# NVIDIA/spark-rapids-ml

Measured on NVIDIA H100. Metric: kmeans_fit_samples_per_sec, higher is better.
Workload: dtype f32

## Files before the change

### profile_fused.py

```python
from __future__ import annotations

import argparse
import json
import os
import sys

ROOT = os.path.dirname(os.path.abspath(__file__))
if ROOT not in sys.path:
    sys.path.insert(0, ROOT)

from bench_pca import _card

CONSUMER = ["X wait", "centre wait", "hand-off wait", "A load + split", "MMA issue + drain", "epilogue", "sort",
            "column sums"]
PRODUCER = ["X slot wait", "centre stage wait", "issue"]
TILE_ROWS = 128


def main() -> None:
    ap = argparse.ArgumentParser()
    ap.add_argument("--rows", type=int, default=10_000_000)
    ap.add_argument("--d", type=int, default=128)
    ap.add_argument("--k", type=int, default=64)
    ap.add_argument("--warmup", type=int, default=3)
    a = ap.parse_args()

    import numpy as np
    import torch

    from bench import make_blobs_device
    from spark_rapids_ml_b200 import _native

    dev = torch.device("cuda", 0)
    X, _ = make_blobs_device(torch, dev, a.rows, a.d, a.k, 0)
    C0 = X[: a.k].clone()
    with _native.Context(0) as ctx:
        ctx.set_option("kernel_path", 2)
        ctx.kmeans_lloyd(X, C0.clone(), a.warmup, -1.0)
        ctx.set_option("profile_fused", 1)
        ctx.kmeans_lloyd(X, C0.clone(), 1, -1.0)
        ctx.set_option("profile_fused", 0)
        prof = ctx.fused_profile().astype(np.float64)
    grid = prof.shape[0]
    ntiles = -(-a.rows // TILE_ROWS)
    tiles = np.array([len(range(b, ntiles, grid)) for b in range(grid)], dtype=np.float64)
    per_tile = prof / tiles[:, None, None]
    cons = per_tile[:, :8, :].mean(axis=(0, 1))
    prod = per_tile[:, 8, :3].mean(axis=0)
    rec = {"shape": {"n": a.rows, "d": a.d, "k": a.k}, "grid": grid, "tiles_per_cta": float(tiles.mean()),
           "consumer_cycles_per_tile": {nm: round(float(v)) for nm, v in zip(CONSUMER, cons)},
           "consumer_total": round(float(cons.sum())),
           "producer_cycles_per_tile": {nm: round(float(v)) for nm, v in zip(PRODUCER, prod)},
           "producer_total": round(float(prod.sum())), **_card()}
    print(f"{rec['gpu']}, power limit {rec['power_limit']}; grid {grid}, {rec['tiles_per_cta']:.1f} tiles per CTA")
    print("consumer warps (mean), cycles per tile:")
    for nm, v in rec["consumer_cycles_per_tile"].items():
        print(f"  {nm:20s} {v:8d}")
    print(f"  {'total':20s} {rec['consumer_total']:8d}")
    print("producer warp, cycles per tile:")
    for nm, v in rec["producer_cycles_per_tile"].items():
        print(f"  {nm:20s} {v:8d}")
    print(f"  {'total':20s} {rec['producer_total']:8d}")
    print(json.dumps(rec))


if __name__ == "__main__":
    main()
```

### spark_rapids_ml_b200/_native.py

```python
from __future__ import annotations

import ctypes
import os
import subprocess
from typing import Any, Dict, List, Optional, Sequence, Tuple

import numpy as np

_PKG_DIR = os.path.dirname(os.path.abspath(__file__))
LIB_PATH = os.environ.get("B2K_LIB") or os.path.join(_PKG_DIR, "libb2kmeans.so")
CSRC_DIR = os.path.join(_PKG_DIR, "csrc")

B2K_OK = 0
INIT_ARRAY, INIT_RANDOM, INIT_KMEANS_PARALLEL = 0, 1, 2
PATH_AUTO, PATH_GENERIC, PATH_FUSED = 0, 1, 2
LAYOUT_ROWS, LAYOUT_COLUMNS = 0, 1
UNIQUE_ID_BYTES = 128

_DTYPE_CODES = {
    np.dtype("float32"): 0,
    np.dtype("float64"): 1,
    np.dtype("int8"): 2,
    np.dtype("int16"): 3,
    np.dtype("int32"): 4,
# ... 203 lines not shown
    L.b2k_dbscan_fit.argtypes = [vp, vp, i64, i32, f64, i32, i32, vp, vp, ctypes.POINTER(i64), ctypes.c_size_t]
    L.b2k_rf_fit.argtypes = [vp, vp, vp, i64, i32, ctypes.POINTER(RfParams), ctypes.POINTER(i32), ctypes.POINTER(i64),
                             vp, vp, ctypes.c_size_t]
    L.b2k_rf_forest.argtypes = [vp, vp, vp, vp, vp, vp, vp, vp]
    L.b2k_rf_predict.argtypes = [vp, vp, i64, i32, i32, vp, vp, vp, vp, vp, i32, i32, vp, vp, vp, ctypes.c_size_t]
    L.b2k_eval_linear.argtypes = [vp, vp, vp, i64, i32, i32, vp, vp, vp, vp, vp, i32, f64, vp, vp, vp, vp, vp,
                                  ctypes.c_size_t]
    L.b2k_eval_forest.argtypes = [vp, vp, vp, i64, i32, i32, i32, vp, vp, vp, vp, vp, vp, vp, i32, f64, vp, vp, vp, vp,
                                  vp, ctypes.c_size_t]
    L.b2k_eval_linear_scores.argtypes = [vp, vp, vp, i64, i32, i32, vp, vp, vp, vp, vp, i64, vp, ctypes.c_size_t]
    L.b2k_eval_forest_scores.argtypes = [vp, vp, vp, i64, i32, i32, vp, vp, vp, vp, vp, vp, vp, vp, i64, vp,
                                         ctypes.c_size_t]
    L.b2k_eval_binary.argtypes = [vp, vp, vp, i64, i32, i32, i32, vp, ctypes.c_size_t]
    L.b2k_umap_fit.argtypes = [vp, vp, i64, i32, vp, ctypes.POINTER(UmapParams), vp, vp, ctypes.c_size_t]
    L.b2k_umap_graph.argtypes = [vp] + [vp] * 11
    L.b2k_umap_transform.argtypes = [vp, vp, vp, i64, i32, vp, i64, ctypes.POINTER(UmapParams), vp, ctypes.c_size_t]
    for name in EXPORTED_SYMBOLS:
        if name not in ("b2k_last_error",):
            getattr(L, name).restype = i32
    _lib = L
    return L


def comm_unique_id() -> bytes:
    L = load_library()
    buf = ctypes.create_string_buffer(UNIQUE_ID_BYTES)
    rc = L.b2k_comm_unique_id(buf)
    if rc != B2K_OK:
        raise B2KError(rc, (L.b2k_last_error(None) or b"").decode())
    return buf.raw


def pca_finalize(cov: np.ndarray, n_total: int, k: int) -> Dict[str, np.ndarray]:
    L = load_library()
    cov = np.ascontiguousarray(cov, dtype=np.float64)
    if cov.ndim != 2 or cov.shape[0] != cov.shape[1]:
        raise ValueError("cov must be a square matrix")
    d = int(cov.shape[0])
    kk = max(int(k), 0)
    comp = np.zeros((kk, d), dtype=np.float64)
    evr = np.zeros(kk, dtype=np.float64)
    sv = np.zeros(kk, dtype=np.float64)
    rc = L.b2k_pca_finalize(cov.ctypes.data, d, int(n_total), int(k), comp.ctypes.data, evr.ctypes.data, sv.ctypes.data)
    if rc != B2K_OK:
        raise B2KError(rc, (L.b2k_last_error(None) or b"").decode())
    return {"components_": comp, "explained_variance_ratio_": evr, "singular_values_": sv}


def linreg_solve(mean: np.ndarray, moments: np.ndarray, n_total: int, reg: float = 0.0, l1_ratio: float = 0.0,
                 fit_intercept: bool = True, standardization: bool = True, max_iter: int = 100,
                 tol: float = 1e-6) -> Tuple[np.ndarray, float, int]:
    L = load_library()
    mean = np.ascontiguousarray(mean, dtype=np.float64)
    moments = np.ascontiguousarray(moments, dtype=np.float64)
    d = int(mean.shape[0]) - 1
    if mean.ndim != 1 or moments.shape != (d + 1, d + 1):
        raise ValueError("mean must be [d + 1] and moments [d + 1, d + 1]")
    coef = np.zeros(max(d, 0), dtype=np.float64)
    b = ctypes.c_double(0.0)
    it = ctypes.c_int(0)
    rc = L.b2k_linreg_solve(mean.ctypes.data, moments.ctypes.data, d, int(n_total), float(reg), float(l1_ratio),
                            int(bool(fit_intercept)), int(bool(standardization)), int(max_iter), float(tol),
                            coef.ctypes.data, ctypes.byref(b), ctypes.byref(it))
    if rc != B2K_OK:
        raise B2KError(rc, (L.b2k_last_error(None) or b"").decode())
    return coef, float(b.value), int(it.value)


def logreg_minimize(fun: Any, x0: np.ndarray, l1: Optional[np.ndarray] = None, max_iter: int = 100,
                    tol: float = 1e-6) -> Tuple[np.ndarray, int, int, float]:
    L = load_library()
    x = np.array(x0, dtype=np.float64, copy=True)
    n = int(x.shape[0])
    l1a = None if l1 is None else np.ascontiguousarray(l1, dtype=np.float64)
    if l1a is not None and l1a.shape != (n,):
        raise ValueError(f"l1 must be [{n}]")
    err: list = []

    def _cb(_user: Any, m: int, xp: Any, fp: Any, gp: Any) -> int:
        try:
            f, g = fun(np.ctypeslib.as_array(xp, shape=(m,)).copy())
            fp[0] = float(f)
            np.ctypeslib.as_array(gp, shape=(m,))[:] = np.asarray(g, dtype=np.float64)
            return 0
        except Exception as e:
            err.append(e)
            return 1

    cb = LOGREG_OBJECTIVE(_cb)
    it, ev, fv = ctypes.c_int(0), ctypes.c_int(0), ctypes.c_double(0.0)
    rc = L.b2k_logreg_minimize(cb, None, n, x.ctypes.data, l1a.ctypes.data if l1a is not None else None,
                               int(max_iter), float(tol), ctypes.byref(it), ctypes.byref(ev), ctypes.byref(fv))
    if err:
        raise err[0]
    if rc != B2K_OK:
        raise B2KError(rc, (L.b2k_last_error(None) or b"").decode())
    return x, int(it.value), int(ev.value), float(fv.value)


def _stream_handle(torch_mod: Any, device: Any) -> int:
    return int(torch_mod.cuda.current_stream(device).cuda_stream)


class Context:

    def __init__(self, device: int = 0):
        import torch

        self._torch = torch
        self._L = load_library()
        self.device_index = int(device)
        self.device = torch.device("cuda", self.device_index)
        h = ctypes.c_void_p()
        rc = self._L.b2k_ctx_create(self.device_index, ctypes.byref(h))
        if rc != B2K_OK:
            raise B2KError(rc, (self._L.b2k_last_error(None) or b"").decode())
        self._h = h
        self.nranks = 1
        self.rank = 0

    def _check(self, rc: int) -> None:
        if rc != B2K_OK:
            raise B2KError(rc, (self._L.b2k_last_error(self._h) or b"").decode())

    def _stream(self) -> int:
        return _stream_handle(self._torch, self.device)

    def close(self) -> None:
        if getattr(self, "_h", None) is not None and self._h:
            self._L.b2k_ctx_destroy(self._h)
            self._h = None

    def __enter__(self) -> "Context":
        return self

    def __exit__(self, *exc: Any) -> None:
        self.close()

    def __del__(self) -> None:
        try:
            self.close()
        except Exception:
            pass

    def set_option(self, key: str, value: int) -> None:
        self._check(self._L.b2k_ctx_set_option(self._h, key.encode(), int(value)))

    def stats(self) -> Dict[str, Any]:
        st = Stats()
        self._check(self._L.b2k_get_stats(self._h, ctypes.byref(st)))
        return {f: getattr(st, f) for f, _ in Stats._fields_}

    def fused_profile(self) -> "np.ndarray":
        buf = np.zeros(1024 * 32 * 8, dtype=np.int64)
        g, w = ctypes.c_int(0), ctypes.c_int(0)
        self._check(self._L.b2k_get_fused_profile(self._h, buf.ctypes.data, buf.size, ctypes.byref(g), ctypes.byref(w)))
        return buf[: g.value * w.value * 8].reshape(g.value, w.value, 8)

    def reset_stats(self) -> None:
        self._check(self._L.b2k_reset_stats(self._h))

    def comm_init(self, nranks: int, rank: int, uid: bytes) -> None:
        assert len(uid) == UNIQUE_ID_BYTES
        self._check(self._L.b2k_comm_init(self._h, int(nranks), int(rank), uid))
        self.nranks, self.rank = int(nranks), int(rank)

    def comm_destroy(self) -> None:
        self._check(self._L.b2k_comm_destroy(self._h))
        self.nranks, self.rank = 1, 0

    def comm_abort(self) -> None:
        self._check(self._L.b2k_comm_abort(self._h))
        self.nranks, self.rank = 1, 0

    def ingest_rows(self, dst: Any, row0: int, values: np.ndarray, d: int,
                    offsets: Optional[np.ndarray] = None, n_rows: Optional[int] = None) -> int:
        code = _DTYPE_CODES.get(values.dtype)
        if code is None:
            raise TypeError(f"unsupported source dtype {values.dtype}")
        assert values.flags.c_contiguous
        if offsets is not None:
            offsets = np.ascontiguousarray(offsets, dtype=np.int32)
            n_b = offsets.shape[0] - 1
        else:
            n_b = int(n_rows) if n_rows is not None else values.size // d
            if values.size != n_b * d:
                raise ValueError(f"feature batch holds {values.size} values for {n_b} rows of width {d}: "
                                 "row width differs from the expected dimension")
        wrote = ctypes.c_int64(0)
        self._check(self._L.b2k_ingest_append(
            self._h, dst.data_ptr(), int(dst.shape[0]), int(d), int(row0), values.ctypes.data,
            offsets.ctypes.data if offsets is not None else None, int(n_b), code, LAYOUT_ROWS,
            self._stream(), ctypes.byref(wrote)))
        return int(wrote.value)

    def ingest_pinned_tensor(self, dst: Any, row0: int, src: Any) -> int:
        assert src.dtype == self._torch.float32 and src.is_contiguous()
        n_b, d = int(src.shape[0]), int(src.shape[1])
        wrote = ctypes.c_int64(0)
        self._check(self._L.b2k_ingest_append(
            self._h, dst.data_ptr(), int(dst.shape[0]), d, int(row0), src.data_ptr(), None, n_b, 0,
            LAYOUT_ROWS, self._stream(), ctypes.byref(wrote)))
        return int(wrote.value)

    def ingest_columns(self, dst: Any, row0: int, columns: Sequence[np.ndarray]) -> int:
        d = len(columns)
        dt = columns[0].dtype
        code = _DTYPE_CODES.get(dt)
        if code is None:
            raise TypeError(f"unsupported source dtype {dt}")
        n_b = int(columns[0].shape[0])
        cols = [np.ascontiguousarray(c) for c in columns]
        for c in cols:
            if c.dtype != dt or c.shape[0] != n_b:
                raise ValueError("columns must share dtype and length")
        ptrs = (ctypes.c_void_p * d)(*[c.ctypes.data for c in cols])
        wrote = ctypes.c_int64(0)
        self._check(self._L.b2k_ingest_append(
            self._h, dst.data_ptr(), int(dst.shape[0]), d, int(row0), ctypes.addressof(ptrs), None, n_b,
            code, LAYOUT_COLUMNS, self._stream(), ctypes.byref(wrote)))
        self._torch.cuda.current_stream(self.device).synchronize()
        return int(wrote.value)

    def _check_X(self, X: Any) -> Tuple[int, int]:
        t = self._torch
        if not (X.is_cuda and X.dtype == t.float32 and X.dim() == 2 and X.is_contiguous()):
            raise ValueError("X must be a contiguous float32 CUDA tensor [n, d]")
        if X.device.index != self.device_index:
            raise ValueError("X lives on a different device than this context")
        return int(X.shape[0]), int(X.shape[1])

    def kmeans_fit(self, X: Any, k: int, *, init: Any = "scalable-k-means++", max_iter: int = 300,
                   tol: float = 1e-4, seed: int = 0, oversampling_factor: float = 2.0, n_init: int = 1,
                   compute_inertia: bool = True) -> Dict[str, Any]:
        t = self._torch
        n, d = self._check_X(X)
        init_ptr = None
        if isinstance(init, str):
            mode = {"scalable-k-means++": INIT_KMEANS_PARALLEL, "k-means||": INIT_KMEANS_PARALLEL,
                    "random": INIT_RANDOM}.get(init)
            if mode is None:
                raise ValueError(f"unknown init {init!r}")
            keep = None
        else:
            keep = t.as_tensor(init, dtype=t.float32, device=self.device).contiguous()
            if tuple(keep.shape) != (k, d):
                raise ValueError(f"init array must have shape ({k}, {d})")
            mode = INIT_ARRAY
            init_ptr = keep.data_ptr()
        centers = t.empty((k, d), dtype=t.float32, device=self.device)
        n_iter = ctypes.c_int(0)
        inertia = ctypes.c_double(0.0)
        with t.cuda.device(self.device):
            self._check(self._L.b2k_kmeans_fit(
                self._h, X.data_ptr(), n, d, int(k), mode, init_ptr, int(max_iter), float(tol),
                int(seed) & 0xFFFFFFFFFFFFFFFF, float(oversampling_factor), int(n_init), centers.data_ptr(),
                ctypes.byref(n_iter), ctypes.byref(inertia) if compute_inertia else None, self._stream()))
        del keep
        return {"cluster_centers_": centers, "n_iter_": int(n_iter.value),
                "inertia_": float(inertia.value) if compute_inertia else None}

    def kmeans_lloyd(self, X: Any, centers: Any, max_iter: int, tol: float) -> Tuple[int, float]:
        t = self._torch
        n, d = self._check_X(X)
        if not (centers.is_cuda and centers.dtype == t.float32 and centers.is_contiguous()
                and centers.shape[1] == d):
            raise ValueError("centers must be a contiguous float32 CUDA tensor [k, d]")
        n_iter = ctypes.c_int(0)
        shift = ctypes.c_double(0.0)
        with t.cuda.device(self.device):
            self._check(self._L.b2k_kmeans_lloyd(
                self._h, X.data_ptr(), n, d, int(centers.shape[0]), centers.data_ptr(), int(max_iter),
                float(tol), ctypes.byref(n_iter), ctypes.byref(shift), self._stream()))
        return int(n_iter.value), float(shift.value)

    def kmeans_assign(self, X: Any, centers: Any, want_mindist: bool = False) -> Tuple[Any, Any]:
        t = self._torch
        n, d = self._check_X(X)
        C = t.as_tensor(centers, dtype=t.float32, device=self.device).contiguous()
        if C.dim() != 2 or C.shape[1] != d:
            raise ValueError("centers must be [k, d]")
        labels = t.empty((n,), dtype=t.int32, device=self.device)
        md = t.empty((n,), dtype=t.float32, device=self.device) if want_mindist else None
        with t.cuda.device(self.device):
            self._check(self._L.b2k_kmeans_assign(
                self._h, X.data_ptr(), n, d, C.data_ptr(), int(C.shape[0]), labels.data_ptr(),
                md.data_ptr() if md is not None else None, self._stream()))
        t.cuda.current_stream(self.device).synchronize()
        return labels, md

    def pca_fit(self, X: Any, k: int) -> Dict[str, np.ndarray]:
        n, d = self._check_X(X)
        kk = max(int(k), 0)
        mean = np.zeros(d, dtype=np.float64)
        comp = np.zeros((kk, d), dtype=np.float64)
        evr = np.zeros(kk, dtype=np.float64)
        sv = np.zeros(kk, dtype=np.float64)
        with self._torch.cuda.device(self.device):
            self._check(self._L.b2k_pca_fit(self._h, X.data_ptr(), n, d, int(k), mean.ctypes.data, comp.ctypes.data,
                                            evr.ctypes.data, sv.ctypes.data, self._stream()))
        return {"mean_": mean, "components_": comp, "explained_variance_ratio_": evr, "singular_values_": sv}

    def pca_transform(self, X: Any, components: Any) -> Any:
        t = self._torch
        n, d = self._check_X(X)
        C = t.as_tensor(components, dtype=t.float32, device=self.device).contiguous()
        if C.dim() != 2 or C.shape[1] != d:
            raise ValueError(f"components must be [k, {d}]")
        k = int(C.shape[0])
        out = t.empty((n, k), dtype=t.float32, device=self.device)
# ... 416 lines not shown
```

### spark_rapids_ml_b200/csrc/b2k_wg.cuh

```cuda
constexpr int WG_TM = B2K_FUSED_TILE_ROWS;
constexpr int WG_CHUNK = 32;
constexpr int WG_XBYTES = WG_TM * WG_CHUNK * 4;
constexpr int WG_NTHREADS = 384;
constexpr int WG_SMEM_LIMIT = 227 * 1024;
constexpr int WG_MISC = 7680;
constexpr int WG_M_CNORM = 256, WG_M_XN = 1280, WG_M_LAB = 1792, WG_M_FLAG = 2816, WG_M_COST = 2880, WG_M_SRT = 2944,
              WG_M_LIST = 3584;
constexpr int WG_MISC3 = 2368;
constexpr int WG_M3_XN = 768, WG_M3_SRT = 768, WG_M3_HIST = 1280, WG_M3_COST = 2304;
constexpr int WG_CL = 8;
constexpr int WG_NPROF = 8;
enum { WG_P_WX, WG_P_WC, WG_P_HAND, WG_P_SPLIT, WG_P_MMA, WG_P_EPI, WG_P_SORT, WG_P_SUMS };

template <int KP, int NCH, bool THREE, bool UPD>
struct WgCfg {
  static_assert(KP % 16 == 0 && KP >= 16 && KP <= 256, "KP");
  static_assert(!UPD || !THREE || (KP <= 128 && NCH <= 4), "3xTF32 covers k, d <= 128");
  static constexpr int SROWS = THREE ? KP : KP / WG_CL;
  static constexpr int DP = NCH * WG_CHUNK;
  static constexpr int NB = THREE ? 2 : 1;
  static constexpr int CBYTES = KP * WG_CHUNK * 4;
  static constexpr int CSTAGE = NB * CBYTES;
  static constexpr int MISC = THREE ? WG_MISC3 : WG_MISC;
  static constexpr int SUM_BYTES = UPD ? SROWS * DP * 4 + SROWS * 4 : 0;
  static constexpr int FIXED = SUM_BYTES + MISC;
  static constexpr int XMIN = UPD ? NCH : 2;
  static constexpr int XRES = UPD ? 2 * NCH : 2;
  static constexpr bool CRES = THREE && (WG_SMEM_LIMIT - FIXED - NCH * CSTAGE) / WG_XBYTES >= XRES;
  static constexpr int SC = CRES ? 1 : (WG_SMEM_LIMIT - FIXED - 2 * CSTAGE) / WG_XBYTES >= XMIN ? 2 : 1;
  static constexpr int C_BYTES = CRES ? NCH * CSTAGE : SC * CSTAGE;
  static constexpr int SX_RAW = (WG_SMEM_LIMIT - FIXED - C_BYTES) / WG_XBYTES;
  static constexpr int SX = SX_RAW > 12 ? 12 : SX_RAW;
  static_assert(SX >= XMIN && 2 * (SX + SC) * 8 + 16 <= WG_M_CNORM, "ring");
  static constexpr int OFF_X = 0;
  static constexpr int OFF_C = SX * WG_XBYTES;
  static constexpr int OFF_SUM = OFF_C + C_BYTES;
  static constexpr int OFF_MISC = OFF_SUM + (THREE ? (SUM_BYTES + 7) & ~7 : (SUM_BYTES + 1023) & ~1023);
  static constexpr int SMEM_BYTES = OFF_MISC + MISC;
  static_assert(SMEM_BYTES <= WG_SMEM_LIMIT, "smem");
  static_assert(!THREE || WG_M_CNORM + KP * 4 <= WG_M3_XN, "misc");
  static_assert(!THREE || WG_M3_HIST + 8 * KP <= WG_M3_COST, "misc");
};
static_assert(WgCfg<64, 4, true, true>::CRES, "cfg2 centres no longer resident");

struct WgArgs {
  int64_t n;
  int ntiles;
  int k;
  int d;
  const float* cnorm;
  int32_t* labels_out;
  float* mind_out;
  double* cost_partials;
  float* partials;
  int32_t* counts;
  const B2kLoopState* st;
  const float* X;
  const float* C32;
  const float* thr;
  const float2* xnorm;
  int2* fix_list;
  uint32_t* fix_masks;
  int32_t* fix_count;
  int seg_cap;
  int mask_cap;
  unsigned long long* rstat;
  long long* prof;
};

__device__ __forceinline__ void wg_merge2(uint32_t& a1, uint32_t& a2, uint32_t b1, uint32_t b2) {
  const uint32_t lo = min(a1, b1), hi = max(a1, b1);
  a2 = min(hi, min(a2, b2));
  a1 = lo;
}

template <int KP, int NCH, bool THREE, bool NC, bool UPD, bool PROF = false>
__global__ void __launch_bounds__(WG_NTHREADS, 1)
k_wg_assign(const __grid_constant__ CUtensorMap mapX, const __grid_constant__ CUtensorMap mapC0,
            const __grid_constant__ CUtensorMap mapC1, const WgArgs args) {
  using G = WgCfg<KP, NCH, THREE, UPD>;
  constexpr int R = KP / 2;
  constexpr int DP = G::DP;
  if (args.st != nullptr && args.st->done) return;

  extern __shared__ __align__(1024) uint8_t smem_raw[];
  const uint32_t base = smem_u32(smem_raw);
  if ((base & 1023u) != 0u) {
    if (threadIdx.x == 0) printf("b2k wgmma: dynamic shared memory base %u is not 1 KB aligned\n", base);
    __trap();
  }
  uint8_t* misc = smem_raw + G::OFF_MISC;
  const uint32_t bars = base + G::OFF_MISC;
  float* cnorm_s = reinterpret_cast<float*>(misc + WG_M_CNORM);
  float* xn_s = reinterpret_cast<float*>(misc + WG_M3_XN);
  int32_t* lab_s = reinterpret_cast<int32_t*>(misc + WG_M_LAB);
  uint8_t* hist_s = misc + WG_M3_HIST;
  int32_t* flag_s = reinterpret_cast<int32_t*>(misc + WG_M_FLAG);
  double* cost_s = reinterpret_cast<double*>(misc + (THREE ? WG_M3_COST : WG_M_COST));
  uint32_t* srt_s = reinterpret_cast<uint32_t*>(misc + (THREE ? WG_M3_SRT : WG_M_SRT));
  float* sum_s = reinterpret_cast<float*>(smem_raw + G::OFF_SUM);
  int32_t* cnt_s = reinterpret_cast<int32_t*>(sum_s + G::SROWS * DP);
  uint32_t* list_s = reinterpret_cast<uint32_t*>(misc + WG_M_LIST);
  auto xfull = [&](int s) -> uint32_t { return bars + 8u * (uint32_t)s; };
  auto xempty = [&](int s) -> uint32_t { return bars + 8u * (uint32_t)(G::SX + s); };
  auto cfull = [&](int s) -> uint32_t { return bars + 8u * (uint32_t)(2 * G::SX + s); };
  auto cempty = [&](int s) -> uint32_t { return bars + 8u * (uint32_t)(2 * G::SX + G::SC + s); };
  constexpr bool CLU = UPD && !THREE;
  const uint32_t ready_bar = bars + 8u * (uint32_t)(2 * G::SX + 2 * G::SC);
  const uint32_t done_bar = ready_bar + 8u;

  const int warp = threadIdx.x >> 5;
  const int lane = threadIdx.x & 31;
  long long pc[WG_NPROF] = {};
  long long tp = PROF ? clock64() : 0;
  auto mark = [&](int ph) {
    if constexpr (PROF) {
      const long long t = clock64();
      pc[ph] += t - tp;
      tp = t;
    }
  };
  auto prof_store = [&]() {
    if constexpr (PROF) {
      long long* o = args.prof + ((size_t)blockIdx.x * (WG_NTHREADS / 32) + warp) * WG_NPROF;
      for (int i = 0; i < WG_NPROF; ++i) o[i] = pc[i];
    }
  };
  if (threadIdx.x == 0) {
    for (int s = 0; s < G::SX; ++s) {
      mbar_init(xfull(s), 1);
      mbar_init(xempty(s), 8);
    }
    for (int s = 0; s < G::SC; ++s) {
      mbar_init(cfull(s), 1);
      mbar_init(cempty(s), 8);
    }
    if constexpr (CLU) {
      mbar_init(ready_bar, WG_CL);
      mbar_init(done_bar, WG_CL);
    }
    asm volatile("fence.mbarrier_init.release.cluster;" ::: "memory");
  }
  for (int j = threadIdx.x; j < KP; j += WG_NTHREADS) cnorm_s[j] = args.cnorm[j];
  if constexpr (UPD) {
    for (int i = threadIdx.x; i < G::SROWS * DP + G::SROWS; i += WG_NTHREADS) sum_s[i] = 0.f;
  }
  __syncthreads();
  uint32_t crank = 0;
  if constexpr (CLU) {
    crank = cluster_ctarank();
    cluster_sync_all();
  }

  const int b0 = (int)blockIdx.x - (int)crank;
  const int nit = b0 < args.ntiles ? (args.ntiles - 1 - b0) / (int)gridDim.x + 1 : 0;

  if (warp >= 8) {
    if constexpr (!THREE) asm volatile("setmaxnreg.dec.sync.aligned.u32 40;" ::: "memory");
    if (warp == 8 && elect_one()) {
      tma_prefetch_desc(&mapX);
      tma_prefetch_desc(&mapC0);
      if constexpr (THREE) tma_prefetch_desc(&mapC1);
      if constexpr (G::CRES) {
        mbar_expect_tx(cfull(0), (uint32_t)(NCH * G::CSTAGE));
        for (int c = 0; c < NCH; ++c) {
          const uint32_t cst = base + (uint32_t)(G::OFF_C + c * G::CSTAGE);
          tma_load_2d(cst, &mapC0, cfull(0), c * WG_CHUNK, 0);
          tma_load_2d(cst + G::CBYTES, &mapC1, cfull(0), c * WG_CHUNK, 0);
        }
      }
      for (int it = 0; it < nit; ++it) {
        const int tile = (int)blockIdx.x + it * (int)gridDim.x;
#pragma unroll 1
        for (int c = 0; c < NCH; ++c) {
          const int q = it * NCH + c;
          const int xs = q % G::SX, cs = q % G::SC;
          mark(WG_P_HAND);
          mbar_wait_nocall(xempty(xs), (uint32_t)((q / G::SX) & 1) ^ 1u);
          mark(WG_P_WX);
          mbar_expect_tx(xfull(xs), (uint32_t)WG_XBYTES);
          tma_load_2d(base + (uint32_t)(G::OFF_X + xs * WG_XBYTES), &mapX, xfull(xs), c * WG_CHUNK, tile * WG_TM);
          if constexpr (!G::CRES) {
            mark(WG_P_HAND);
            mbar_wait_nocall(cempty(cs), (uint32_t)((q / G::SC) & 1) ^ 1u);
            mark(WG_P_WC);
            const uint32_t cst = base + (uint32_t)(G::OFF_C + cs * G::CSTAGE);
            mbar_expect_tx(cfull(cs), (uint32_t)G::CSTAGE);
            tma_load_2d(cst, &mapC0, cfull(cs), c * WG_CHUNK, 0);
            if constexpr (THREE) tma_load_2d(cst + G::CBYTES, &mapC1, cfull(cs), c * WG_CHUNK, 0);
          }
        }
      }
      mark(WG_P_HAND);
      prof_store();
    }
    __syncwarp();
  } else {
    if constexpr (!THREE) asm volatile("setmaxnreg.inc.sync.aligned.u32 232;" ::: "memory");
    const int g = warp >> 2, wi = warp & 3, tw = threadIdx.x & 127;
    float acc[R];
#pragma unroll
    for (int i = 0; i < R; ++i) acc[i] = 0.f;
    double cost = 0.0;
    int seg_cnt = 0;
    unsigned long long n_flag = 0;
    float thr0 = 0.f, thr1 = 0.f, thr2 = 0.f, thr3 = 0.f;
    if constexpr (!THREE) {
      thr0 = args.thr[0];
      thr1 = args.thr[1];
      thr2 = args.thr[2];
      thr3 = args.thr[3];
    }
    if constexpr (THREE) {
      const uint32_t arow = (uint32_t)(g * 64 + wi * 16 + (lane >> 2)) * 128u + (uint32_t)(lane & 3) * 4u;
      const uint32_t asw = (uint32_t)(lane >> 2);
      constexpr bool PIPE = (G::CRES || G::SC > 1) && KP < 128;
      if constexpr (G::CRES) {
        mark(WG_P_EPI);
        if (nit > 0) mbar_wait_nocall(cfull(0), 0u);
        mark(WG_P_WC);
      }
      for (int it = 0; it < nit; ++it) {
        const int tile = (int)blockIdx.x + it * (int)gridDim.x;
        float xnp[4] = {0.f, 0.f, 0.f, 0.f};
#pragma unroll
        for (int c = 0; c < NCH; ++c) {
          const int q = it * NCH + c;
          const int xsl = q % G::SX, csl = q % G::SC;
          const uint32_t xs = base + (uint32_t)(G::OFF_X + xsl * WG_XBYTES);
          const uint32_t cs = base + (uint32_t)(G::OFF_C + (G::CRES ? c : csl) * G::CSTAGE);
          const uint8_t* xp = smem_raw + G::OFF_X + xsl * WG_XBYTES;
          mark(WG_P_EPI);
          mbar_wait_nocall(xfull(xsl), (uint32_t)((q / G::SX) & 1));
          mark(WG_P_WX);
          if constexpr (NC) {
#pragma unroll
            for (int i = 0; i < 4; ++i) {
              const float4 v = lds128(xs + (uint32_t)(g * (WG_XBYTES / 2) + (tw + 128 * i) * 16));
              xnp[i] = fmaf(v.w, v.w, fmaf(v.z, v.z, fmaf(v.y, v.y, fmaf(v.x, v.x, xnp[i]))));
            }
          }
          uint32_t ah[WG_CHUNK / 8][4], al[WG_CHUNK / 8][4];
#pragma unroll
          for (int ks = 0; ks < WG_CHUNK / 8; ++ks) {
#pragma unroll
            for (int e = 0; e < 4; ++e) {
              const uint32_t unit = (uint32_t)(2 * ks + (e >> 1));
              const float v = *reinterpret_cast<const float*>(xp + arow + (uint32_t)(e & 1) * 1024u + ((unit ^ asw) << 4));
              ah[ks][e] = rn_tf32_bits(v);
              al[ks][e] = rn_tf32_bits(v - __uint_as_float(ah[ks][e]));
            }
          }
#pragma unroll
          for (int ks = 0; ks < WG_CHUNK / 8; ++ks) {
            reg_fence(ah[ks]);
            reg_fence(al[ks]);
          }
          if constexpr (!UPD) {
            __syncwarp();
            if (lane == 0) mbar_arrive(xempty(xsl));
          }
          mark(WG_P_SPLIT);
          if constexpr (!G::CRES) {
            mbar_wait_nocall(cfull(csl), (uint32_t)((q / G::SC) & 1));
            mark(WG_P_WC);
          }
          wgmma_fence();
#pragma unroll
          for (int ks = 0; ks < WG_CHUNK / 8; ++ks) {
            const uint64_t db = make_kmajor_sw128_desc(cs + ks * 32);
            const uint64_t dbl = make_kmajor_sw128_desc(cs + G::CBYTES + ks * 32);
            wgmma_tf32_rs<KP>(acc, al[ks], db, (c | ks) != 0 ? 1u : 0u);
            wgmma_tf32_rs<KP>(acc, ah[ks], dbl, 1u);
            wgmma_tf32_rs<KP>(acc, ah[ks], db, 1u);
          }
          wgmma_commit();
          if constexpr (PIPE) {
            wgmma_wait1();
            if constexpr (!G::CRES) {
              if (c > 0) {
                __syncwarp();
                if (lane == 0) mbar_arrive(cempty((q - 1) % G::SC));
              }
            }
          } else {
            wgmma_wait0();
            if constexpr (!G::CRES) {
              __syncwarp();
              if (lane == 0) mbar_arrive(cempty(csl));
            }
          }
          mark(WG_P_MMA);
        }
        wgmma_wait0();
        if constexpr (PIPE && !G::CRES) {
          __syncwarp();
          if (lane == 0) mbar_arrive(cempty((it * NCH + NCH - 1) % G::SC));
        }
        reg_fence(acc);
        mark(WG_P_MMA);

        const int rr0 = g * 64 + wi * 16 + (lane >> 2);
        if constexpr (NC) {
#pragma unroll
          for (int i = 0; i < 4; ++i) {
            float v = xnp[i];
            v += __shfl_xor_sync(0xffffffffu, v, 1);
            v += __shfl_xor_sync(0xffffffffu, v, 2);
            v += __shfl_xor_sync(0xffffffffu, v, 4);
            if ((lane & 7) == 0) xn_s[g * 64 + (tw >> 3) + 16 * i] = v;
          }
          asm volatile("bar.sync %0, 128;" ::"r"(1 + g) : "memory");
        }
        float best[2] = {__int_as_float(0x7f800000), __int_as_float(0x7f800000)};
        int bj[2] = {0, 0};
#pragma unroll
        for (int i = 0; i < R; ++i) {
          const int h = (i >> 1) & 1;
          const int j = (i >> 2) * 8 + 2 * (lane & 3) + (i & 1);
          const float dist = fmaf(-2.f, acc[i], cnorm_s[j]);
          if (dist < best[h]) { best[h] = dist; bj[h] = j; }
        }
#pragma unroll
        for (int h = 0; h < 2; ++h) {
#pragma unroll
          for (int o = 1; o <= 2; o <<= 1) {
            const float ob = __shfl_xor_sync(0xffffffffu, best[h], o);
            const int oj = __shfl_xor_sync(0xffffffffu, bj[h], o);
            if (ob < best[h] || (ob == best[h] && oj < bj[h])) { best[h] = ob; bj[h] = oj; }
          }
          const int64_t grow = (int64_t)tile * WG_TM + rr0 + 8 * h;
          if ((lane & 3) == 0) {
            if (grow < args.n) {
              if (args.labels_out != nullptr) args.labels_out[grow] = bj[h];
              if constexpr (NC) {
                const float md = fmaxf(xn_s[rr0 + 8 * h] + best[h], 0.f);
                if (args.mind_out != nullptr) args.mind_out[grow] = md;
                cost += (double)md;
              }
            }
          }
        }
        mark(WG_P_EPI);
        if constexpr (UPD) {
          const int hq = lane & 3;
          const int64_t grow0 = (int64_t)tile * WG_TM + rr0;
          const uint32_t key = hq == 0   ? (grow0 < args.n ? (uint32_t)bj[0] : (uint32_t)KP)
                               : hq == 1 ? (grow0 + 8 < args.n ? (uint32_t)bj[1] : (uint32_t)KP)
                                         : 0x10000u + (uint32_t)lane;
          const bool own = hq < 2 && key < (uint32_t)KP;
          const uint32_t mk = __match_any_sync(0xffffffffu, key);
          const uint32_t lt = (1u << lane) - 1u;
          const int wr = hq == 0 ? __popc(mk & 0x11111111u & lt) : __popc(mk & 0x11111111u) + __popc(mk & 0x22222222u & lt);
          uint8_t* hist = hist_s + warp * KP;
          if (lane < KP / 4) reinterpret_cast<uint32_t*>(hist)[lane] = 0u;
          __syncwarp();
          if (own && wr == 0) hist[key] = (uint8_t)__popc(mk & 0x33333333u);
          mark(WG_P_SORT);
          asm volatile("bar.sync 3, 256;" ::: "memory");
          mark(WG_P_HAND);
          uint32_t tot = 0u, pre = 0u;
          if (lane < KP / 4) {
#pragma unroll
            for (int w = 0; w < 8; ++w) {
              const uint32_t v = reinterpret_cast<const uint32_t*>(hist_s + w * KP)[lane];
              tot += v;
              if (w < warp) pre += v;
            }
          }
          const int lsum = (int)((tot * 0x01010101u) >> 24);
          int incl = lsum;
#pragma unroll
          for (int o = 1; o < 32; o <<= 1) {
            const int v = __shfl_up_sync(0xffffffffu, incl, o);
            if (lane >= o) incl += v;
          }
          const int nv = __shfl_sync(0xffffffffu, incl, 31);
          const uint32_t first = tot * 0x01010100u + (uint32_t)(incl - lsum) * 0x01010101u + pre;
          const uint32_t fb = __shfl_sync(0xffffffffu, first, (int)(key >> 2) & 31);
          if (own) srt_s[((fb >> (8 * (key & 3u))) & 0xffu) + (uint32_t)wr] = (key << 16) | (uint32_t)(rr0 + 8 * hq);
          mark(WG_P_SORT);
          asm volatile("bar.sync 3, 256;" ::: "memory");
          mark(WG_P_HAND);
          int p0 = 128, p1 = 128;
          {
            const uint4 e4 = *reinterpret_cast<const uint4*>(srt_s + 4 * lane);
            const uint32_t ev[4] = {e4.x, e4.y, e4.z, e4.w};
            uint32_t prev = __shfl_up_sync(0xffffffffu, e4.w >> 16, 1);
#pragma unroll
            for (int i = 0; i < 4; ++i) {
              const int p = 4 * lane + i;
              const uint32_t l = ev[i] >> 16;
              if (p < nv && (p == 0 || l != prev)) {
                if (p >= 16 * warp && p0 == 128) p0 = p;
                if (p >= 16 * warp + 16 && p1 == 128) p1 = p;
              }
              prev = l;
            }
            p0 = min(__reduce_min_sync(0xffffffffu, p0), nv);
            p1 = min(__reduce_min_sync(0xffffffffu, p1), nv);
          }
          const bool act = lane < DP / 4;
          const uint8_t* xbase = smem_raw + G::OFF_X + ((it * NCH + (act ? lane >> 3 : 0)) % G::SX) * WG_XBYTES;
          const uint32_t unit = (uint32_t)(lane & 7);
          float4 a = make_float4(0.f, 0.f, 0.f, 0.f);
          int cur = -1, run = 0;
          auto flush = [&]() {
            if (act) {
              float4* sp = reinterpret_cast<float4*>(sum_s + cur * DP) + lane;
              float4 s = *sp;
              s.x += a.x;
              s.y += a.y;
              s.z += a.z;
              s.w += a.w;
              *sp = s;
            }
            if (lane == 0) cnt_s[cur] += run;
          };
#pragma unroll 1
          for (int i0 = p0; i0 < p1; i0 += 8) {
            uint32_t e[8];
            float4 x[8];
#pragma unroll
            for (int v = 0; v < 8; ++v) e[v] = i0 + v < p1 ? srt_s[i0 + v] : 0xffffffffu;
#pragma unroll
            for (int v = 0; v < 8; ++v) {
              const uint32_t r = e[v] & 127u;
              x[v] = *reinterpret_cast<const float4*>(xbase + r * 128u + ((unit ^ (r & 7u)) << 4));
            }
#pragma unroll
            for (int v = 0; v < 8; ++v) {
              if (e[v] == 0xffffffffu) break;
              const int l = (int)(e[v] >> 16);
              if (l != cur) {
                if (cur >= 0) flush();
                cur = l;
                a = make_float4(0.f, 0.f, 0.f, 0.f);
                run = 0;
              }
              a.x += x[v].x;
              a.y += x[v].y;
              a.z += x[v].z;
              a.w += x[v].w;
              ++run;
            }
          }
          if (cur >= 0) flush();
          __syncwarp();
          if (lane == 0) {
#pragma unroll
            for (int c = 0; c < NCH; ++c) mbar_arrive(xempty((it * NCH + c) % G::SX));
          }
          mark(WG_P_SUMS);
        }
      }
    } else {
      for (int it = 0; it < nit; ++it) {
        const int tile = (int)blockIdx.x + it * (int)gridDim.x;
        int prev_q = -1;
#pragma unroll 1
        for (int c = 0; c < NCH; ++c) {
          const int q = it * NCH + c;
          const int xsl = q % G::SX, csl = q % G::SC;
          const uint32_t xs = base + (uint32_t)(G::OFF_X + xsl * WG_XBYTES + g * (WG_XBYTES / 2));
          const uint32_t cs = base + (uint32_t)(G::OFF_C + csl * G::CSTAGE);
          mbar_wait_nocall(xfull(xsl), (uint32_t)((q / G::SX) & 1));
          mbar_wait_nocall(cfull(csl), (uint32_t)((q / G::SC) & 1));
          wgmma_fence();
#pragma unroll
          for (int ks = 0; ks < WG_CHUNK / 8; ++ks) {
            const uint64_t da = make_kmajor_sw128_desc(xs + ks * 32);
            const uint64_t db = make_kmajor_sw128_desc(cs + ks * 32);
            const uint32_t sd = (c | ks) != 0 ? 1u : 0u;
            wgmma_tf32<KP>(acc, da, db, sd);
          }
          wgmma_commit();
          if constexpr (G::SC == 1) {
            wgmma_wait0();
            __syncwarp();
            if (lane == 0) {
              mbar_arrive(cempty(csl));
              if constexpr (!UPD) mbar_arrive(xempty(xsl));
            }
          } else {
            wgmma_wait1();
            if (prev_q >= 0) {
              __syncwarp();
              if (lane == 0) {
                if constexpr (!UPD) mbar_arrive(xempty(prev_q % G::SX));
                mbar_arrive(cempty(prev_q % G::SC));
              }
            }
            prev_q = q;
          }
        }
        if constexpr (G::SC > 1) {
          wgmma_wait0();
          __syncwarp();
          if (lane == 0) {
            if constexpr (!UPD) mbar_arrive(xempty(prev_q % G::SX));
            mbar_arrive(cempty(prev_q % G::SC));
          }
        }
        reg_fence(acc);

        const int rr0 = g * 64 + wi * 16 + (lane >> 2);
        float thr[2], xoff[2];
        bool valid[2];
        int64_t grow[2];
#pragma unroll
        for (int h = 0; h < 2; ++h) {
          grow[h] = (int64_t)tile * WG_TM + rr0 + 8 * h;
          valid[h] = grow[h] < args.n;
          const float2 xq = valid[h] ? __ldg(args.xnorm + grow[h]) : make_float2(0.f, 0.f);
          thr[h] = fmaf(xq.y, thr0, fmaf(xq.x, fmaf(xq.x, thr2, thr1), thr3));
          xoff[h] = fmaf(xq.x, xq.x, thr[h]);
        }
        uint32_t m1[2] = {0xffffffffu, 0xffffffffu}, m2[2] = {0xffffffffu, 0xffffffffu};
#pragma unroll
        for (int i = 0; i < R; ++i) {
          const int h = (i >> 1) & 1;
          const int j = (i >> 2) * 8 + 2 * (lane & 3) + (i & 1);
          const float dist = fmaf(-2.f, acc[i], cnorm_s[j]) + xoff[h];
          const uint32_t key = (__float_as_uint(dist) & 0xffffff00u) | (uint32_t)j;
          wg_merge2(m1[h], m2[h], key, 0xffffffffu);
        }
        bool flag[2];
        int label[2];
        float T[2];
#pragma unroll
        for (int h = 0; h < 2; ++h) {
#pragma unroll
          for (int o = 1; o <= 2; o <<= 1) {
            const uint32_t r1 = __shfl_xor_sync(0xffffffffu, m1[h], o), r2 = __shfl_xor_sync(0xffffffffu, m2[h], o);
            wg_merge2(m1[h], m2[h], r1, r2);
          }
          label[h] = (int)(m1[h] & 255u);
          const float M1f = __uint_as_float(m1[h] & 0xffffff00u);
          flag[h] = valid[h] && (__uint_as_float(m2[h] & 0xffffff00u) - M1f) < thr[h];
          T[h] = M1f + thr[h];
        }
        const uint32_t b0 = __ballot_sync(0xffffffffu, flag[0] && (lane & 3) == 0);
        const uint32_t b1 = __ballot_sync(0xffffffffu, flag[1] && (lane & 3) == 0);
        const int pb = it & 1;
        if (lane == 0) flag_s[pb * 8 + warp] = __popc(b0) + __popc(b1);
        if ((lane & 3) == 0) {
#pragma unroll
          for (int h = 0; h < 2; ++h) lab_s[pb * WG_TM + rr0 + 8 * h] = (valid[h] && !flag[h]) ? label[h] : -1;
        }
        uint32_t mk[2][KP / 32];
#pragma unroll
        for (int h = 0; h < 2; ++h)
#pragma unroll
          for (int w = 0; w < KP / 32; ++w) mk[h][w] = 0u;
        if (__any_sync(0xffffffffu, flag[0] || flag[1])) {
#pragma unroll
          for (int i = 0; i < R; ++i) {
            const int h = (i >> 1) & 1;
            const int j = (i >> 2) * 8 + 2 * (lane & 3) + (i & 1);
            const float dist = fmaf(-2.f, acc[i], cnorm_s[j]) + xoff[h];
            if (__uint_as_float(__float_as_uint(dist) & 0xffffff00u) <= T[h]) mk[h][i >> 4] |= 1u << (j & 31);
          }
#pragma unroll
          for (int h = 0; h < 2; ++h)
#pragma unroll
            for (int w = 0; w < KP / 32; ++w) {
              mk[h][w] |= __shfl_xor_sync(0xffffffffu, mk[h][w], 1);
              mk[h][w] |= __shfl_xor_sync(0xffffffffu, mk[h][w], 2);
            }
        }
        asm volatile("bar.sync 3, 256;" ::: "memory");
        int pre = 0, total = 0;
#pragma unroll
        for (int w = 0; w < 8; ++w) {
          const int v = flag_s[pb * 8 + w];
          if (w < warp) pre += v;
          total += v;
        }
        if ((lane & 3) == 0) {
          const uint32_t lt = (1u << lane) - 1u;
#pragma unroll
          for (int h = 0; h < 2; ++h) {
            if (flag[h]) {
              const int e = seg_cnt + pre + (h == 0 ? __popc(b0 & lt) : __popc(b0) + __popc(b1 & lt));
              args.fix_list[(size_t)blockIdx.x * (size_t)args.seg_cap + e] = make_int2((int)grow[h], -1);
              if (e < args.mask_cap) {
                uint32_t* dst = args.fix_masks + ((size_t)blockIdx.x * (size_t)args.mask_cap + (size_t)e) * 8u;
#pragma unroll
                for (int w = 0; w < 8; ++w) dst[w] = w < KP / 32 ? mk[h][w < KP / 32 ? w : 0] : 0u;
              }
              ++n_flag;
            } else if (valid[h] && args.labels_out != nullptr) {
              args.labels_out[grow[h]] = label[h];
            }
          }
        }
        seg_cnt += total;
        if constexpr (CLU) {
          constexpr int SR = G::SROWS;
          const uint32_t par = (uint32_t)(it & 1);
          if (threadIdx.x == 0) {
            for (int r = 0; r < WG_CL; ++r) mbar_arrive_remote(ready_bar, (uint32_t)r);
          }
          mbar_wait_cluster_nocall(ready_bar, par);
          const uint32_t lab_src = mapa_u32(smem_u32(lab_s + pb * WG_TM), (uint32_t)warp);
          uint32_t m[4];
          int rel[4], n_my = 0;
// ... 167 lines not shown
```

Before: 3.528 billion.

## Defer per-cluster column sums one tile to overlap with MMA work

In the 3xTF32 update path, the column-sum accumulation for tile it-1 now runs while the next tile's MMAs are in flight. Warpgroup 0 does it before issuing, warpgroup 1 after the wait, and the last tile is flushed after the loop. This hides the sums latency behind tensor-core work but holds X slots one tile longer, which requires SX >= 2*NCH. The profiler also splits MMA issue from MMA wait.

Measured after the change: 3.643 billion, median of 6. +3.3%, better.

```diff
diff --git a/profile_fused.py b/profile_fused.py
--- a/profile_fused.py
+++ b/profile_fused.py
@@ -11,8 +11,8 @@
 
 from bench_pca import _card
 
-CONSUMER = ["X wait", "centre wait", "hand-off wait", "A load + split", "MMA issue + drain", "epilogue", "sort",
-            "column sums"]
+CONSUMER = ["X wait", "centre wait", "hand-off wait", "A load + split", "MMA issue", "epilogue", "sort",
+            "column sums", "MMA wait"]
 PRODUCER = ["X slot wait", "centre stage wait", "issue"]
 TILE_ROWS = 128
 
diff --git a/spark_rapids_ml_b200/_native.py b/spark_rapids_ml_b200/_native.py
--- a/spark_rapids_ml_b200/_native.py
+++ b/spark_rapids_ml_b200/_native.py
@@ -379,10 +379,10 @@
         return {f: getattr(st, f) for f, _ in Stats._fields_}
 
     def fused_profile(self) -> "np.ndarray":
-        buf = np.zeros(1024 * 32 * 8, dtype=np.int64)
+        buf = np.zeros(1024 * 32 * 9, dtype=np.int64)
         g, w = ctypes.c_int(0), ctypes.c_int(0)
         self._check(self._L.b2k_get_fused_profile(self._h, buf.ctypes.data, buf.size, ctypes.byref(g), ctypes.byref(w)))
-        return buf[: g.value * w.value * 8].reshape(g.value, w.value, 8)
+        return buf[: g.value * w.value * 9].reshape(g.value, w.value, 9)
 
     def reset_stats(self) -> None:
         self._check(self._L.b2k_reset_stats(self._h))
diff --git a/spark_rapids_ml_b200/csrc/b2k_wg.cuh b/spark_rapids_ml_b200/csrc/b2k_wg.cuh
--- a/spark_rapids_ml_b200/csrc/b2k_wg.cuh
+++ b/spark_rapids_ml_b200/csrc/b2k_wg.cuh
@@ -9,8 +9,8 @@
 constexpr int WG_MISC3 = 2368;
 constexpr int WG_M3_XN = 768, WG_M3_SRT = 768, WG_M3_HIST = 1280, WG_M3_COST = 2304;
 constexpr int WG_CL = 8;
-constexpr int WG_NPROF = 8;
-enum { WG_P_WX, WG_P_WC, WG_P_HAND, WG_P_SPLIT, WG_P_MMA, WG_P_EPI, WG_P_SORT, WG_P_SUMS };
+constexpr int WG_NPROF = 9;
+enum { WG_P_WX, WG_P_WC, WG_P_HAND, WG_P_SPLIT, WG_P_MMA, WG_P_EPI, WG_P_SORT, WG_P_SUMS, WG_P_MMAW };
 
 template <int KP, int NCH, bool THREE, bool UPD>
 struct WgCfg {
@@ -32,6 +32,7 @@
   static constexpr int SX_RAW = (WG_SMEM_LIMIT - FIXED - C_BYTES) / WG_XBYTES;
   static constexpr int SX = SX_RAW > 12 ? 12 : SX_RAW;
   static_assert(SX >= XMIN && 2 * (SX + SC) * 8 + 16 <= WG_M_CNORM, "ring");
+  static constexpr bool OVL = THREE && UPD && SX >= 2 * NCH;
   static constexpr int OFF_X = 0;
   static constexpr int OFF_C = SX * WG_XBYTES;
   static constexpr int OFF_SUM = OFF_C + C_BYTES;
@@ -42,6 +43,8 @@
   static_assert(!THREE || WG_M3_HIST + 8 * KP <= WG_M3_COST, "misc");
 };
 static_assert(WgCfg<64, 4, true, true>::CRES, "cfg2 centres no longer resident");
+static_assert(WgCfg<64, 4, true, true>::OVL, "cfg2 sums no longer overlapped");
+static_assert(!WgCfg<128, 4, true, true>::OVL, "KP = DP = 128 now fits the overlapped schedule");
 
 struct WgArgs {
   int64_t n;
@@ -215,14 +218,73 @@
       const uint32_t arow = (uint32_t)(g * 64 + wi * 16 + (lane >> 2)) * 128u + (uint32_t)(lane & 3) * 4u;
       const uint32_t asw = (uint32_t)(lane >> 2);
       constexpr bool PIPE = (G::CRES || G::SC > 1) && KP < 128;
+      constexpr bool OVL = G::OVL;
       if constexpr (G::CRES) {
         mark(WG_P_EPI);
         if (nit > 0) mbar_wait_nocall(cfull(0), 0u);
         mark(WG_P_WC);
       }
+      const bool act = lane < DP / 4;
+      const uint32_t unit = (uint32_t)(lane & 7);
+      int p0 = 0, p1 = 0;
+      const uint8_t* xsum = smem_raw;
+      auto sums = [&](int its) {
+        float4 a = make_float4(0.f, 0.f, 0.f, 0.f);
+        int cur = -1, run = 0;
+        auto flush = [&]() {
+          if (act) {
+            float4* sp = reinterpret_cast<float4*>(sum_s + cur * DP) + lane;
+            float4 s = *sp;
+            s.x += a.x;
+            s.y += a.y;
+            s.z += a.z;
+            s.w += a.w;
+            *sp = s;
+          }
+          if (lane == 0) cnt_s[cur] += run;
+        };
+#pragma unroll 1
+        for (int i0 = p0; i0 < p1; i0 += 8) {
+          uint32_t e[8];
+          float4 x[8];
+#pragma unroll
+          for (int v = 0; v < 8; ++v) e[v] = i0 + v < p1 ? srt_s[i0 + v] : 0xffffffffu;
+#pragma unroll
+          for (int v = 0; v < 8; ++v) {
+            const uint32_t r = e[v] & 127u;
+            x[v] = *reinterpret_cast<const float4*>(xsum + r * 128u + ((unit ^ (r & 7u)) << 4));
+          }
+#pragma unroll
+          for (int v = 0; v < 8; ++v) {
+            if (e[v] == 0xffffffffu) break;
+            const int l = (int)(e[v] >> 16);
+            if (l != cur) {
+              if (cur >= 0) flush();
+              cur = l;
+              a = make_float4(0.f, 0.f, 0.f, 0.f);
+              run = 0;
+            }
+            a.x += x[v].x;
+            a.y += x[v].y;
+            a.z += x[v].z;
+            a.w += x[v].w;
+            ++run;
+          }
+        }
+        if (cur >= 0) flush();
+        __syncwarp();
+        if (lane == 0) {
+#pragma unroll
+          for (int c = 0; c < NCH; ++c) mbar_arrive(xempty((its * NCH + c) % G::SX));
+        }
+      };
       for (int it = 0; it < nit; ++it) {
         const int tile = (int)blockIdx.x + it * (int)gridDim.x;
         float xnp[4] = {0.f, 0.f, 0.f, 0.f};
+        if constexpr (OVL) {
+          if (g == 0 && it > 0) sums(it - 1);
+          mark(WG_P_SUMS);
+        }
 #pragma unroll
         for (int c = 0; c < NCH; ++c) {
           const int q = it * NCH + c;
@@ -275,6 +337,7 @@
             wgmma_tf32_rs<KP>(acc, ah[ks], db, 1u);
           }
           wgmma_commit();
+          mark(WG_P_MMA);
           if constexpr (PIPE) {
             wgmma_wait1();
             if constexpr (!G::CRES) {
@@ -290,7 +353,7 @@
               if (lane == 0) mbar_arrive(cempty(csl));
             }
           }
-          mark(WG_P_MMA);
+          mark(WG_P_MMAW);
         }
         wgmma_wait0();
         if constexpr (PIPE && !G::CRES) {
@@ -298,7 +361,11 @@
           if (lane == 0) mbar_arrive(cempty((it * NCH + NCH - 1) % G::SC));
         }
         reg_fence(acc);
-        mark(WG_P_MMA);
+        mark(WG_P_MMAW);
+        if constexpr (OVL) {
+          if (g == 1 && it > 0) sums(it - 1);
+          mark(WG_P_SUMS);
+        }
 
         const int rr0 = g * 64 + wi * 16 + (lane >> 2);
         if constexpr (NC) {
@@ -382,8 +449,8 @@
           mark(WG_P_SORT);
           asm volatile("bar.sync 3, 256;" ::: "memory");
           mark(WG_P_HAND);
-          int p0 = 128, p1 = 128;
           {
+            int q0 = 128, q1 = 128;
             const uint4 e4 = *reinterpret_cast<const uint4*>(srt_s + 4 * lane);
             const uint32_t ev[4] = {e4.x, e4.y, e4.z, e4.w};
             uint32_t prev = __shfl_up_sync(0xffffffffu, e4.w >> 16, 1);
@@ -392,67 +459,24 @@
               const int p = 4 * lane + i;
               const uint32_t l = ev[i] >> 16;
               if (p < nv && (p == 0 || l != prev)) {
-                if (p >= 16 * warp && p0 == 128) p0 = p;
-                if (p >= 16 * warp + 16 && p1 == 128) p1 = p;
+                if (p >= 16 * warp && q0 == 128) q0 = p;
+                if (p >= 16 * warp + 16 && q1 == 128) q1 = p;
               }
               prev = l;
             }
-            p0 = min(__reduce_min_sync(0xffffffffu, p0), nv);
-            p1 = min(__reduce_min_sync(0xffffffffu, p1), nv);
-          }
-          const bool act = lane < DP / 4;
-          const uint8_t* xbase = smem_raw + G::OFF_X + ((it * NCH + (act ? lane >> 3 : 0)) % G::SX) * WG_XBYTES;
-          const uint32_t unit = (uint32_t)(lane & 7);
-          float4 a = make_float4(0.f, 0.f, 0.f, 0.f);
-          int cur = -1, run = 0;
-          auto flush = [&]() {
-            if (act) {
-              float4* sp = reinterpret_cast<float4*>(sum_s + cur * DP) + lane;
-              float4 s = *sp;
-              s.x += a.x;
-              s.y += a.y;
-              s.z += a.z;
-              s.w += a.w;
-              *sp = s;
-            }
-            if (lane == 0) cnt_s[cur] += run;
-          };
-#pragma unroll 1
-          for (int i0 = p0; i0 < p1; i0 += 8) {
-            uint32_t e[8];
-            float4 x[8];
-#pragma unroll
-            for (int v = 0; v < 8; ++v) e[v] = i0 + v < p1 ? srt_s[i0 + v] : 0xffffffffu;
-#pragma unroll
-            for (int v = 0; v < 8; ++v) {
-              const uint32_t r = e[v] & 127u;
-              x[v] = *reinterpret_cast<const float4*>(xbase + r * 128u + ((unit ^ (r & 7u)) << 4));
-            }
-#pragma unroll
-            for (int v = 0; v < 8; ++v) {
-              if (e[v] == 0xffffffffu) break;
-              const int l = (int)(e[v] >> 16);
-              if (l != cur) {
-                if (cur >= 0) flush();
-                cur = l;
-                a = make_float4(0.f, 0.f, 0.f, 0.f);
-                run = 0;
-              }
-              a.x += x[v].x;
-              a.y += x[v].y;
-              a.z += x[v].z;
-              a.w += x[v].w;
-              ++run;
-            }
-          }
-          if (cur >= 0) flush();
-          __syncwarp();
-          if (lane == 0) {
-#pragma unroll
-            for (int c = 0; c < NCH; ++c) mbar_arrive(xempty((it * NCH + c) % G::SX));
-          }
-          mark(WG_P_SUMS);
-        }
+            p0 = min(__reduce_min_sync(0xffffffffu, q0), nv);
+            p1 = min(__reduce_min_sync(0xffffffffu, q1), nv);
+          }
+          xsum = smem_raw + G::OFF_X + ((it * NCH + (act ? lane >> 3 : 0)) % G::SX) * WG_XBYTES;
+          if constexpr (!OVL) {
+            sums(it);
+            mark(WG_P_SUMS);
+          }
+        }
+      }
+      if constexpr (OVL) {
+        if (nit > 0) sums(nit - 1);
+        mark(WG_P_SUMS);
       }
     } else {
       for (int it = 0; it < nit; ++it) {
```
